# mika314/melonix

Hardware: AMD Instinct MI355X
Metric: STFT+pitch+resynth frames/sec (48 kHz, 4096 FFT, 256 hop); % HBM roofline (higher is better)
Workload: dtype f32

## Files before the change

melonix_amd/csrc/capi_ctx.cpp:

```cpp
#include "capi_internal.h"
#include "stft_tables.h"

using namespace mx;

namespace mx {
namespace {
thread_local char g_err[512] = "";
}
int fail(int code, const char *fmt, ...) noexcept {
  va_list ap;
  va_start(ap, fmt);
  vsnprintf(g_err, sizeof(g_err), fmt, ap);
  va_end(ap);
  return code;
}

int default_frames_per_block(int N, int mode, int hop, int64_t count) {
  if (const char *e = getenv("MELONIX_FRAMES_PER_BLOCK")) {
    const int v = atoi(e);
    if (v > 0) return v;
  }
  const int cap = stft_frames_per_block_cap(N, mode, hop);
  const int64_t want_blocks = 2048;
  const int64_t want = std::max<int64_t>(1, std::min<int64_t>(cap, count / want_blocks));
  int g = 1;
  while (2 * g <= want) g *= 2;
  return g;
}

template <class P>
int build_tables(NTables &t) {
  constexpr int N = P::N;
  const auto tw2 = make_tw2<P>();
  const auto tw3 = make_tw3<P>();
  const auto ub = make_ubase<P>();
  HIP_TRY(hipMalloc(&t.tw2, tw2.size() * sizeof(float2)));
  HIP_TRY(hipMalloc(&t.tw3, tw3.size() * sizeof(float2)));
  HIP_TRY(hipMalloc(&t.ubase, ub.size() * sizeof(float2)));
  HIP_TRY(hipMemcpy(t.tw2, tw2.data(), tw2.size() * sizeof(float2), hipMemcpyHostToDevice));
  HIP_TRY(hipMemcpy(t.tw3, tw3.data(), tw3.size() * sizeof(float2), hipMemcpyHostToDevice));
  HIP_TRY(hipMemcpy(t.ubase, ub.data(), ub.size() * sizeof(float2), hipMemcpyHostToDevice));
  t.wext_host = make_wext(fold_scale(N));
  HIP_TRY(hipMalloc(&t.wext, t.wext_host.size() * sizeof(float)));
  HIP_TRY(hipMemcpy(t.wext, t.wext_host.data(), t.wext_host.size() * sizeof(float), hipMemcpyHostToDevice));
  return MX_OK;
}

int get_tables(mx_ctx *ctx, int N, NTables &out) {
  std::lock_guard<std::mutex> lk(ctx->mu);
  auto it = ctx->tables.find(N);
  if (it != ctx->tables.end()) {
    out = it->second;
    return MX_OK;
  }
  NTables t;
  int rc;
  switch (N) {
    case 4096: rc = build_tables<Plan<4096, kPlan4096E>>(t); break;
    case 16384: rc = build_tables<Plan<16384, 32>>(t); break;
    case 32768: rc = build_tables<Plan<32768, 32>>(t); break;
    default: return fail(MX_ERR_INVALID, "unsupported FFT size %d (supported: 4096, 16384, 32768)", N);
  }
  if (rc) return rc;
  ctx->tables[N] = t;
  out = t;
  return MX_OK;
}

int get_wtab(mx_ctx *ctx, int N, int hop, const NTables &nt, const float **out) {
  std::lock_guard<std::mutex> lk(ctx->mu);
  const auto key = std::make_pair(N, hop);
  auto it = ctx->wtabs.find(key);
  if (it != ctx->wtabs.end()) {
    *out = it->second;
    return MX_OK;
  }
  const std::vector<float> w = make_wtab(N, hop, nt.wext_host);
  float *d = nullptr;
  HIP_TRY(hipMalloc(&d, w.size() * sizeof(float)));
  HIP_TRY(hipMemcpy(d, w.data(), w.size() * sizeof(float), hipMemcpyHostToDevice));
  ctx->wtabs[key] = d;
  *out = d;
  return MX_OK;
}

int check_common(mx_ctx *ctx, const mx_audio *a, int N, int64_t count, int &kmin, int &kmax) {
  if (!ctx || !a) return fail(MX_ERR_INVALID, "null context or audio handle");
  if (N != 4096 && N != 16384 && N != 32768)
    return fail(MX_ERR_INVALID, "unsupported FFT size %d (supported: 4096, 16384, 32768)", N);
  if (count < 0) return fail(MX_ERR_INVALID, "negative frame count");
  if (kmin < 0 && kmax < 0) mx_pitch_band(N, 48000, &kmin, &kmax);
  kmin = std::max(kmin, 0);
  kmax = std::min(kmax, N / 2 - 1);
  if (kmin > kmax) return fail(MX_ERR_INVALID, "empty pitch band [%d,%d]", kmin, kmax);
  return MX_OK;
}

int stft_launch(mx_ctx *ctx, const mx_audio *a, int N, int mode, int hop, int64_t first_frame,
                const int32_t *d_ranges, int64_t count, int kmin, int kmax, float *d_mags,
                mx_pitch *d_pitch, uint8_t *d_rgb, float cmap_k, int run_length) {
  HIP_TRY(hipSetDevice(ctx->device));
  NTables t;
  int rc = get_tables(ctx, N, t);
  if (rc) return rc;
  StftArgs s{};
  s.audio = a->d_padded;
  s.n = a->n;
  s.wext = t.wext;
  s.decay = hop_decay(hop);
  s.tw2 = t.tw2;
  s.tw3 = t.tw3;
  s.ubase = t.ubase;
  s.ranges = d_ranges;
  s.hop = hop;
  s.first_frame = first_frame;
  s.count = count;
  s.kmin = kmin;
  s.kmax = kmax;
  s.mags = d_mags;
  s.pitch = d_pitch;
  s.rgb = d_rgb;
  s.cmap_k = cmap_k;
  s.frames_per_block = (mode != kRanges && ctx->frames_per_block > 0) ? ctx->frames_per_block
                       : run_length > 0                              ? run_length
                                                                     : default_frames_per_block(N, mode, hop, count);
  if (mode != kRanges) {
    rc = get_wtab(ctx, N, hop, t, &s.wtab);
    if (rc) return rc;
  }
  HIP_TRY(launch_stft(N, mode, s, ctx->stream));
  return MX_OK;
}

int64_t chunk_frames(int N) { return std::max<int64_t>(1, (int64_t)(1ull << 30) / ((int64_t)(N / 2) * 4)); }

void stage_trim(mx_ctx *ctx) {
  for (auto &st : ctx->stage)
    if (st.cap > ((size_t)256 << 20)) st.drop();
}

}

extern "C" {

const char *mx_last_error(void) { return g_err; }
#ifndef MX_SRC_SHA
#define MX_SRC_SHA "unknown"
#endif
const char *mx_version(void) { return "melonix_amd 0.1.0 gfx950 src:" MX_SRC_SHA; }

int mx_ctx_create(int device, mx_ctx **out) {
  return mx_guard([&]() -> int {
    if (!out) return fail(MX_ERR_INVALID, "out is null");
    *out = nullptr;
    int ndev = 0;
    hipError_t e = hipGetDeviceCount(&ndev);
    if (e != hipSuccess || ndev <= 0)
      return fail(MX_ERR_DEVICE, "no HIP device visible (%s); melonix_amd has no CPU path",
                  e == hipSuccess ? "device count is 0" : hipGetErrorString(e));
    if (device < 0 || device >= ndev) return fail(MX_ERR_INVALID, "device %d out of range [0,%d)", device, ndev);
    hipDeviceProp_t prop;
    HIP_TRY(hipGetDeviceProperties(&prop, device));
    if (strncmp(prop.gcnArchName, "gfx950", 6) != 0)
      return fail(MX_ERR_DEVICE, "device %d is %s; this library carries gfx950 (MI355X) code objects only", device,
                  prop.gcnArchName);
    HIP_TRY(hipSetDevice(device));
    mx_ctx *c = new (std::nothrow) mx_ctx();
    if (!c) return fail(MX_ERR_NOMEM, "out of host memory");
    c->device = device;
    e = hipStreamCreateWithFlags(&c->own_stream, hipStreamNonBlocking);
    if (e != hipSuccess) {
      delete c;
      return fail(MX_ERR_DEVICE, "hipStreamCreate: %s", hipGetErrorString(e));
    }
    c->stream = c->own_stream;
    *out = c;
    return MX_OK;
  });
}

void mx_ctx_destroy(mx_ctx *ctx) {
  mx_guard_void([&] {
    if (!ctx) return;
    hipSetDevice(ctx->device);
    hipStreamSynchronize(ctx->stream);
    for (auto &kv : ctx->tables) {
      hipFree(kv.second.tw2);
      hipFree(kv.second.tw3);
      hipFree(kv.second.ubase);
      hipFree(kv.second.wext);
    }
    for (auto &kv : ctx->wtabs) hipFree(kv.second);
    for (auto &st : ctx->stage) st.drop();
    for (auto &st : ctx->chain) st.drop();
    for (auto &st : ctx->f0dec) st.drop();
    pv_release(ctx);
    hipStreamDestroy(ctx->own_stream);
    delete ctx;
  });
}

int mx_ctx_set_stream(mx_ctx *ctx, void *hip_stream) {
  return mx_guard([&]() -> int {
    if (!ctx) return fail(MX_ERR_INVALID, "null context");
    ctx->stream = (hipStream_t)hip_stream;
    return MX_OK;
  });
}

int mx_ctx_use_own_stream(mx_ctx *ctx) {
  return mx_guard([&]() -> int {
    if (!ctx) return fail(MX_ERR_INVALID, "null context");
    ctx->stream = ctx->own_stream;
    return MX_OK;
  });
}

int mx_ctx_synchronize(mx_ctx *ctx) {
  return mx_guard([&]() -> int {
    if (!ctx) return fail(MX_ERR_INVALID, "null context");
    HIP_TRY(hipStreamSynchronize(ctx->stream));
    return MX_OK;
  });
}

int mx_ctx_release_scratch(mx_ctx *ctx) {
  return mx_guard([&]() -> int {
    if (!ctx) return fail(MX_ERR_INVALID, "null context");
    HIP_TRY(hipSetDevice(ctx->device));
    {
      std::lock_guard<std::mutex> lk(ctx->stage_mu);
      for (auto &st : ctx->stage) st.drop();
    }
    {
      std::lock_guard<std::mutex> lk(ctx->pv_mu);
      pv_release(ctx);
      ctx->pv_budget_auto = 0;
      ctx->pv_rec_full = false;
    }
    {
      std::lock_guard<std::mutex> lk(ctx->zc_mu);
      ctx->zc_scratch = ZcBitmaps{};
      for (auto &st : ctx->chain) st.drop();
    }
    {
      std::lock_guard<std::mutex> lk(ctx->f0_mu);
      for (auto &st : ctx->f0dec) st.drop();
    }
    return MX_OK;
  });
}

int mx_pinned_alloc(mx_ctx *ctx, size_t bytes, void **out) {
  return mx_guard([&]() -> int {
    if (!ctx || !out) return fail(MX_ERR_INVALID, "null context / out");
    *out = nullptr;
    if (bytes == 0) return MX_OK;
    HIP_TRY(hipSetDevice(ctx->device));
    const hipError_t e = hipHostMalloc(out, bytes, hipHostMallocDefault);
    if (e != hipSuccess) {
      *out = nullptr;
      return fail(MX_ERR_NOMEM, "hipHostMalloc(%zu): %s", bytes, hipGetErrorString(e));
    }
    return MX_OK;
  });
}

void mx_pinned_free(mx_ctx *ctx, void *p) {
  mx_guard_void([&] {
    if (!p) return;
    if (ctx) hipSetDevice(ctx->device);
    hipHostFree(p);
  });
}

int mx_ctx_set_frames_per_block(mx_ctx *ctx, int g) {
  return mx_guard([&]() -> int {
    if (!ctx || g < 0) return fail(MX_ERR_INVALID, "bad argument");
    ctx->frames_per_block = g;
    return MX_OK;
  });
}

int mx_audio_upload(mx_ctx *ctx, const float *host_wav, int64_t n, mx_audio **out) {
  return mx_guard([&]() -> int {
    if (!ctx || !out || n < 0 || (n > 0 && !host_wav)) return fail(MX_ERR_INVALID, "bad argument");
    if (n > 0x7fffffffLL - 2 * MX_AUDIO_PAD)
      return fail(MX_ERR_INVALID, "audio longer than the reference's int sample indices allow");
    HIP_TRY(hipSetDevice(ctx->device));
    mx_audio *a = new (std::nothrow) mx_audio();
    if (!a) return fail(MX_ERR_NOMEM, "out of host memory");
    const size_t total = (size_t)n + 2 * (size_t)MX_AUDIO_PAD;
    hipError_t e = hipMalloc(&a->d_padded, total * sizeof(float));
    if (e == hipSuccess) e = hipMemsetAsync(a->d_padded, 0, total * sizeof(float), ctx->stream);
    if (e == hipSuccess && n > 0)
      e = hipMemcpyAsync(a->d_padded + MX_AUDIO_PAD, host_wav, (size_t)n * sizeof(float), hipMemcpyHostToDevice,
                         ctx->stream);
    if (e == hipSuccess) e = hipStreamSynchronize(ctx->stream);
    if (e != hipSuccess) {
      if (a->d_padded) hipFree(a->d_padded);
      delete a;
      return fail(MX_ERR_DEVICE, "audio upload: %s", hipGetErrorString(e));
    }
    a->n = n;
    a->owned = true;
    *out = a;
    return MX_OK;
  });
}

int mx_audio_wrap_device(mx_ctx *ctx, const float *d_padded, int64_t n, mx_audio **out) {
  return mx_guard([&]() -> int {
    if (!ctx || !out || !d_padded || n < 0) return fail(MX_ERR_INVALID, "bad argument");
    if (reinterpret_cast<uintptr_t>(d_padded) & 15)
      return fail(MX_ERR_INVALID, "device audio buffer must be 16-byte aligned");
    mx_audio *a = new (std::nothrow) mx_audio();
    if (!a) return fail(MX_ERR_NOMEM, "out of host memory");
    a->d_padded = const_cast<float *>(d_padded);
    a->n = n;
    a->owned = false;
    *out = a;
    return MX_OK;
  });
}

int64_t mx_audio_length(const mx_audio *a) {
  return mx_guard([&]() -> int64_t {
    return a ? a->n : -1;
  });
}

int mx_audio_free(mx_ctx *ctx, mx_audio *a) {
  return mx_guard([&]() -> int {
    if (!a) return MX_OK;
    if (a->owned) {
      if (ctx) {
        hipSetDevice(ctx->device);
        hipStreamSynchronize(ctx->stream);
      }
      hipFree(a->d_padded);
    }
    delete a;
    return MX_OK;
  });
}
void mx_free(void *p) {
  mx_guard_void([&] {
    free(p);
  });
}

}
```

melonix_amd/csrc/kernels.h:

```cpp
#pragma once
#include <hip/hip_runtime.h>
#include <stdint.h>

#include "../../include/melonix_amd.h"

namespace mx {

enum StftMode {
  kBulkAligned = 0,
  kBulkAny = 1,
  kRanges = 2,
};

struct StftArgs {
  const float *audio;
  int64_t n;
  const float *wtab;
  const float *wext;
  float decay;
  const float2 *tw2;
  const float2 *tw3;
  const float2 *ubase;
  const int32_t *ranges;
  int hop;
  int64_t first_frame;
  int64_t count;
  int kmin, kmax;
  float *mags;
  mx_pitch *pitch;
  uint8_t *rgb;
  float cmap_k;
  int frames_per_block;
};

hipError_t launch_stft(int N, int mode, const StftArgs &a, hipStream_t s);
constexpr int kPlan4096E = 16;
int stft_points_per_thread(int N);
int stft_frames_per_block_cap(int N, int mode, int hop);

struct ResynthArgs {
  const float *audio;
  const mx_step *steps;
  int64_t nsteps;
  int64_t nsamples;
  float *pcm_f32;
  int16_t *pcm_i16;
};
hipError_t launch_resynth(const ResynthArgs &a, hipStream_t s);

struct PvArgs {
  const float *audio;
  int64_t n;
  double ratio;
  const int64_t *apos;
  const uint32_t *hop;
  const double *hratio;
  int64_t frames;
  const float *hann_scaled;
  const float *hann;
  const float2 *wsplit;
  const float2 *tw2, *tw3, *ubase;
  float2 *xrows;
  uint32_t *pkmap;
  uint32_t *pkcount;
  float *fthr;
  uint2 *recs;
  uint32_t rec_wg_cap;
  int rec_fpb_shift;
  uint32_t *rec_overflow;
  uint32_t *chunk_sums;
  uint16_t *chunk_org;
  uint32_t *group_sums;
  uint16_t *group_org;
  int scan_chunk;
  float *halo;
  float *s;
  int64_t s_len;
  float *pcm_f32;
  int16_t *pcm_i16;
  int64_t pcm_base;
  int frames_per_block;
  int64_t first;
  int global_first;
  const uint32_t *carry_in;
  uint32_t *carry_out;
  uint32_t *tot_sums;
  uint16_t *tot_org;
  const float *prev_tail;
  const float *next_head;
  const float *prev_final;
  int skip_head, skip_tail;
  int64_t out_lo, out_hi;
  int64_t s_origin;
  const double *tf, *rf;
  const int64_t *i0;
  int64_t frame_base;
  int sample_rate;
};
hipError_t launch_pv(const PvArgs &a, hipStream_t s);
hipError_t launch_pv_analyze(const PvArgs &a, hipStream_t s);
hipError_t launch_pv_synthesize(const PvArgs &a, hipStream_t s);
hipError_t launch_pv_analysis(const PvArgs &a, hipStream_t s);
hipError_t launch_pv_maps(const PvArgs &a, hipStream_t s);
hipError_t launch_pv_offsets(const PvArgs &a, hipStream_t s);
hipError_t launch_pv_synthesis(const PvArgs &a, hipStream_t s);
hipError_t launch_pv_finish(const PvArgs &a, hipStream_t s);
int64_t pv_halo_floats(int64_t frames);
hipError_t launch_pv_compose_maps(const uint32_t *sums, const uint16_t *org, int64_t n, uint32_t *out_sums, uint16_t *out_org, hipStream_t s,
                                  int sums_stride = 0, int org_stride = 0);
hipError_t launch_pv_resample(const PvArgs &a, hipStream_t s);
hipError_t launch_pv_edge_sum(float *dst, const float *x, const float *y, int n, hipStream_t s);
hipError_t launch_pv_plan_const(int64_t *apos, uint32_t *hop, double *hratio, int64_t rows, int64_t fbase, double r,
                                hipStream_t s);

struct F0Args {
  const float *audio;
  int hop;
  int64_t first_frame;
  int64_t count;
  int tau_min, tau_max;
  float threshold;
  const float2 *tw2, *tw3, *ubase;
  mx_f0 *out;
  int frames_per_block;
  mx_f0_cand *cands;
  int sample_rate;
};
hipError_t launch_f0(const F0Args &a, hipStream_t s);

struct F0DecodeArgs {
  const mx_f0 *track;
  const mx_f0_cand *cands;
  int64_t count;
  int64_t q_unvoiced, q_jump, q_switch;
  int32_t max_jump_cents;
  int64_t chunk;
  uint16_t *bp;
  int64_t *prod;
  uint16_t *map;
  mx_f0 *out;
  uint8_t *state;
};
int64_t f0_decode_default_chunk(int64_t count);
hipError_t launch_f0_decode(const F0DecodeArgs &a, hipStream_t s);
hipError_t launch_colormap(const float *mags, uint8_t *rgb, int64_t nbins_total, float k, hipStream_t s);

hipError_t launch_picks(const float *audio_padded, int64_t n, float *d_out, int64_t *counts, int *nlevels, hipStream_t s);

hipError_t launch_zc_bitmaps(const float *audio_padded, int64_t n, uint64_t *zc7, uint64_t *zc3,
                             hipStream_t s);

size_t grain_rank_scratch_bytes(int64_t n);
hipError_t launch_grain_rank(const float *audio_padded, int64_t n, const uint64_t *zc7, const uint64_t *zc3, void *rank_scratch,
                             hipStream_t s);
void grain_chain_sizes(int64_t n, uint32_t nodes, int *levels_out, uint32_t *out_cap_out, size_t *bytes_out);
hipError_t launch_grain_chain(const float *audio_padded, int64_t n, const uint64_t *zc7, const uint64_t *zc3, void *rank_scratch,
                              uint32_t nodes, void *chain_scratch, int32_t **d_starts, int32_t **d_lens, float **d_firsts,
                              hipStream_t s);

}
```

melonix_amd/csrc/stft_kernel_impl.h:

```cpp
#pragma once
#include <hip/hip_runtime.h>

#include "colormap_core.h"
#include "kernels.h"
#include "stft_core.h"
#include "stft_tables.h"

#define MX_BARRIER() __syncthreads()

namespace mx {

template <bool MAXOP>
__device__ __forceinline__ unsigned wave_reduce_u32(unsigned k) {
  constexpr unsigned ident = MAXOP ? 0u : 0xffffffffu;
#define MX_DPP_STEP(CTRL, ROWS)                                                                      \
  {                                                                                                  \
    const unsigned o = (unsigned)__builtin_amdgcn_update_dpp((int)ident, (int)k, CTRL, ROWS, 0xf, false); \
    k = MAXOP ? (o > k ? o : k) : (o < k ? o : k);                                                   \
  }
  MX_DPP_STEP(0xB1, 0xf)
  MX_DPP_STEP(0x4E, 0xf)
  MX_DPP_STEP(0x141, 0xf)
  MX_DPP_STEP(0x140, 0xf)
  MX_DPP_STEP(0x142, 0xa)
  MX_DPP_STEP(0x143, 0xc)
#undef MX_DPP_STEP
  return (unsigned)__builtin_amdgcn_readlane((int)k, 63);
}
__device__ __forceinline__ unsigned long long wave_max_u64(unsigned long long k) {
  const unsigned hi = (unsigned)(k >> 32), lo = (unsigned)k;
  const unsigned mhi = wave_reduce_u32<true>(hi);
  const unsigned long long tie = __ballot(hi == mhi);
  unsigned mlo;
  if (__builtin_popcountll(tie) == 1) mlo = (unsigned)__builtin_amdgcn_readlane((int)lo, __builtin_ctzll(tie));
  else mlo = wave_reduce_u32<true>(hi == mhi ? lo : 0u);
  return ((unsigned long long)mhi << 32) | mlo;
}

template <int IMM, bool NT = true>
__device__ __forceinline__ void st_row_nt(const float *base, unsigned off, float x) {
  static_assert(IMM >= -4096 && IMM <= 4095, "global_store immediate offset");
#if defined(__HIP_DEVICE_COMPILE__)
  if constexpr (NT) asm volatile("global_store_dword %0, %1, %2 offset:%3 nt" : : "v"(off), "v"(x), "s"(base), "n"(IMM) : "memory");
  else asm volatile("global_store_dword %0, %1, %2 offset:%3" : : "v"(off), "v"(x), "s"(base), "n"(IMM) : "memory");
#endif
}

template <class P, int MODE, int HOP, int WPE, bool DEFER = false, bool PREFETCH = false, bool CMAP = false, bool DIRECT = false,
          bool CIRC = false>
__global__ __launch_bounds__(P::T) __attribute__((amdgpu_waves_per_eu(WPE, WPE)))
void stft_kernel(const StftArgs a0) {
  const StftArgs &a = a0;
  using C = P;
  constexpr int N = P::N;
  constexpr int NW = C::T / 64;
  constexpr int kRed = (NW > 1) ? ((NW + 1) / 2) * 2 : 0;
  constexpr bool kTw3Bases = (P::R3 == 16);
  constexpr int kTw2 = ((C::TW2 + 1) / 2) * 2;
  static_assert(P::R3 == 16 || P::R3 == 8, "twiddle placement per plan");
  static_assert(!DIRECT || (NW > 1 && !DEFER && !CMAP), "direct row stores: multi-wave, non-deferred plans");
  static_assert(!CIRC || (MODE != kRanges && HOP == 0 && !PREFETCH && !CMAP), "circular window: bulk modes");
  constexpr int IMG = t1_size<C>();
  __shared__ __attribute__((aligned(16))) float2 lds[IMG + kRed + (DEFER ? C::M / 2 : 0) + kTw2];
  float *const lout = reinterpret_cast<float *>(DEFER ? lds + IMG + kRed : lds);
  float2 *const ltw2 = lds + IMG + kRed + (DEFER ? C::M / 2 : 0);

  const int t_ = threadIdx.x;
  const bool wave0 = __builtin_amdgcn_readfirstlane(t_) < 64;
  cpx u[kTw3Bases ? 1 : P::R3];
  cpx ulo;
  cpx w3r[kTw3Bases ? 1 : P::R3 - 1], w3base[6];
  if constexpr (kTw3Bases) {
    cpx uhi_unused;
    post_bases<P>(t_, a.ubase, ulo, uhi_unused);
    fetch_tw3_bases<P>(t_, a.tw3, w3base);
  } else {
    post_twiddles<P>(t_, a.ubase, *reinterpret_cast<cpx(*)[P::R3]>(&u));
    fetch_tw3<P>(t_, a.tw3, *reinterpret_cast<cpx(*)[P::R3 - 1]>(&w3r));
  }
  const uint32_t bmask_ = band_mask<P>(t_, a.kmin, a.kmax);
  uint32_t umask = 0;
#pragma unroll
  for (int o = 0; o < P::E; ++o) umask |= (__ballot((bmask_ >> o) & 1u) != 0ull) ? (1u << o) : 0u;
  umask = __builtin_amdgcn_readfirstlane(umask);
  constexpr bool kSlide = (MODE == kBulkAligned) && (HOP > 0) && Slide<P, (HOP > 0 ? HOP : 2)>::ok;
  constexpr int SD = Slide<P, (HOP > 0 ? HOP : 2)>::D;
  constexpr float kSc = 0.5f / (float)N;
  for (int i = t_; i < C::TW2; i += C::T) ltw2[i] = a.tw2[i];
  MX_BARRIER();

  unsigned lb = blockIdx.x;
  {
    const unsigned nb = gridDim.x, xcd = lb & 7u, q = nb >> 3, r = nb & 7u;
    lb = (xcd < r ? xcd * (q + 1) : r * (q + 1) + (xcd - r) * q) + (lb >> 3);
  }
  const int64_t f0 = (int64_t)lb * a.frames_per_block;
  const int64_t f1 = (f0 + a.frames_per_block < a.count) ? f0 + a.frames_per_block : a.count;

  cpx Y[P::E];
  cpx edge[SD], nx[SD];
  if constexpr (kSlide) {
    const int64_t e0 = (a.first_frame + f0 + 1) * (int64_t)HOP;
    if (f0 < f1) load_frame<P, 1, true>(t_, Y, a.audio + MX_AUDIO_PAD + (e0 - N), a.wtab);
    slide_edge<P, HOP>(t_, a.wtab, 2.0f * (float)N, edge);
  }

  unsigned long long *const red = reinterpret_cast<unsigned long long *>(lds + IMG);
  auto flush_pitch = [&](int64_t fr, int tt) {
    if (a.pitch && tt == 0) {
      unsigned long long b = red[0];
#pragma unroll
      for (int i = 1; i < NW; ++i) b = red[i] > b ? red[i] : b;
      mx_pitch p;
      p.bin = 0x7fffffff - (int)(unsigned)(b & 0xffffffffull);
      p.mag = __uint_as_float((unsigned)(b >> 32));
      a.pitch[fr] = p;
    }
  };
  const bool want_rows = a.mags != nullptr || (CMAP && a.rgb != nullptr);
  auto flush_row = [&](int64_t fr, int tt) {
    if (want_rows) {
      using f32x4 = float __attribute__((ext_vector_type(4)));
      const f32x4 *l4 = reinterpret_cast<const f32x4 *>(lout) + tt;
      f32x4 *row4 = reinterpret_cast<f32x4 *>(a.mags + (size_t)fr * (size_t)(N / 2)) + tt;
      f32x4 q[C::M / 4 / C::T];
#pragma unroll
      for (int i = 0; i < C::M / 4 / C::T; ++i) q[i] = l4[C::T * i];
      if (!CMAP || a.mags) {
#pragma unroll
        for (int i = 0; i < C::M / 4 / C::T; ++i) {
          __builtin_nontemporal_store(q[i], &row4[C::T * i]);
        }
      }
      if constexpr (CMAP) {
        if (a.rgb) {
          uint32_t *trow = reinterpret_cast<uint32_t *>(a.rgb + (size_t)fr * (size_t)(N / 2) * 3) + 3 * tt;
#pragma unroll 1
          for (int i = 0; i < C::M / 4 / C::T; ++i) {
            uint32_t w3[3];
            texel4(q[i].x, q[i].y, q[i].z, q[i].w, a.cmap_k, w3);
            uint32_t *o = trow + 3 * C::T * i;
            o[0] = w3[0];
            o[1] = w3[1];
            o[2] = w3[2];
          }
        }
      }
    }
  };

  auto frame_ptrs = [&](int64_t fr, int zo, const float *&x, const float *&w) {
    if constexpr (MODE == kRanges) {
      const int s = a.ranges[2 * fr], e = a.ranges[2 * fr + 1];
      const bool outside = (e <= 0) || ((int64_t)e - N >= a.n);
      x = outside ? a.audio : a.audio + MX_AUDIO_PAD + ((int64_t)e - N);
      int64_t d0 = (int64_t)N - ((int64_t)e - (int64_t)s);
      d0 = d0 < (int64_t)(N - 1 - kWOff) ? (int64_t)(N - 1 - kWOff) : d0;
      d0 = d0 > (int64_t)(kWDmax + kWTail) ? (int64_t)(kWDmax + kWTail) : d0;
      w = a.wext + kWOff + d0;
    } else {
      const int64_t e = (a.first_frame + fr + 1) * (int64_t)a.hop;
      x = a.audio + MX_AUDIO_PAD + (e - N);
      w = a.wtab + zo;
    }
  };
  float cpx_[2 * Circ<P>::CS], cpw_[2 * Circ<P>::CS];
  if constexpr (CIRC) {
    if (f0 < f1) {
      const int64_t pe = (a.first_frame + f0 + 1) * (int64_t)a.hop;
      circ_load_first<P>(t_, Y, a.audio + MX_AUDIO_PAD + (pe - N), a.wtab, circ_geo<P>(pe, a.hop).o);
    }
  }
  cpx xr[(PREFETCH && !kSlide) ? P::E : 1];
  if constexpr (PREFETCH && !kSlide) {
    if (f0 < f1) {
      const float *x0;
      const float *w0;
      frame_ptrs(f0, 0, x0, w0);
      load_raw<P, (MODE == kBulkAligned)>(t_, xr, x0);
    }
  }

  for (int64_t f = f0; f < f1; ++f) {
    int t = t_;
    unsigned bmask = bmask_;
    int zoff = 0;
    asm volatile("" : "+v"(t), "+v"(bmask), "+s"(zoff));
    int out_lo, out_hi;
    out_bases<P>(t, out_lo, out_hi);

    if constexpr (CIRC) {
      if (f > f0) {
        const int64_t pe = (a.first_frame + f + 1) * (int64_t)a.hop;
        const CircGeo<P> geo = circ_geo<P>(pe, a.hop);
        circ_fetch<P>(t, a.audio + MX_AUDIO_PAD + (pe - 2 * (int64_t)a.hop), a.wtab + zoff + (N - 2 * a.hop), geo, cpx_, cpw_);
        circ_step<P>(t, Y, a.decay, geo, cpx_, cpw_);
      }
    } else if constexpr (kSlide) {
      if (f > f0) slide_step<P, HOP>(Y, nx, edge, a.decay, kSc);
      if (f + 1 < f1) slide_fetch<P, HOP>(t, a.audio + MX_AUDIO_PAD + (a.first_frame + f + 2) * (int64_t)HOP, nx);
    } else {
      const float *x;
      const float *w;
      frame_ptrs(f, zoff, x, w);
      if constexpr (PREFETCH) {
        if constexpr (MODE == kRanges) apply_window<P, -1, false>(t, Y, xr, w);
        else apply_window_geo<P>(t, Y, xr, a.wtab + N + zoff, a.hop);
      } else if constexpr (MODE == kRanges) {
        load_frame<P, -1, false>(t, Y, x, w);
      } else {
        load_frame_geo<P, (MODE == kBulkAligned)>(t, Y, x, a.wtab + N + zoff, a.hop);
      }
    }

    cpx v[P::E];
    pass1<P>(Y, v);
    constexpr bool kTw2Batch = (P::NB2 == 1);
    store_t1<P>(t, v, lds);
    MX_BARRIER();
    if constexpr (DEFER || DIRECT) {
      if (f > f0) flush_pitch(f - 1, t);
    }
    if constexpr (kTw2Batch) {
      cpx w2[P::R2 - 1];
      load_t1_tw2<P>(t, v, lds, ltw2, w2);
      if constexpr (DEFER) {
        if (f > f0) flush_row(f - 1, t);
      }
      MX_BARRIER();
      pass2_reg<P>(v, w2);
    } else {
      load_t1<P>(t, v, lds);
      if constexpr (DEFER) {
        if (f > f0) flush_row(f - 1, t);
      }
      MX_BARRIER();
      pass2<P>(t, v, ltw2);
    }
    store_t2<P>(t, v, lds);
    MX_BARRIER();
    load_t2<P>(t, v, lds);
    MX_BARRIER();
    float mg[P::E];
    if (NW == 1 || wave0) {
      if constexpr (kTw3Bases) {
        pass3_bases<P, true>(t, v, w3base);
        post_fly<P, true>(t, v, ulo, csel(t == 0, mk(-1.0f, 0.0f), ulo), mg);
      } else {
        pass3_reg<P, true>(t, v, *reinterpret_cast<cpx(*)[P::R3 - 1]>(&w3r));
        post<P, true>(t, v, *reinterpret_cast<cpx(*)[P::R3]>(&u), mg);
      }
    } else {
      if constexpr (kTw3Bases) {
        pass3_bases<P, false>(t, v, w3base);
        post_fly<P, false>(t, v, ulo, ulo, mg);
      } else {
        pass3_reg<P, false>(t, v, *reinterpret_cast<cpx(*)[P::R3 - 1]>(&w3r));
        post<P, false>(t, v, *reinterpret_cast<cpx(*)[P::R3]>(&u), mg);
      }
    }

    if constexpr (PREFETCH && !kSlide) {
      if (f + 1 < f1) {
        const float *xn;
        const float *wn;
        frame_ptrs(f + 1, zoff, xn, wn);
        load_raw<P, (MODE == kBulkAligned)>(t, xr, xn);
      }
    }

    unsigned long long best = 0ull;
    if (a.pitch) {
      const unsigned klo = 0x7fffffffu - (unsigned)out_lo, khi = 0x7fffffffu - (unsigned)out_hi;
      const unsigned nlo = 0x7fffffffu - (unsigned)(C::M - out_lo), nhi = 0x7fffffffu - (unsigned)(C::M - out_hi);
#pragma unroll
      for (int s = 0; s < C::R3; ++s) {
        constexpr int H = C::R3 / 2;
        if (!((umask >> (2 * s)) & 3u)) continue;
        const unsigned b0 = (s < H ? klo : khi) - (unsigned)(C::NS3 * s);
        unsigned b1 = (s < H ? nlo : nhi) + (unsigned)(C::NS3 * s);
        if (s == H) b1 = (t == 0) ? 0x7fffffffu - (unsigned)(C::M / 2) : b1;
        const unsigned v0 = (unsigned)((int)(bmask << (31 - 2 * s)) >> 31);
        const unsigned v1 = (unsigned)((int)(bmask << (31 - (2 * s + 1))) >> 31);
        const unsigned long long k0 = ((unsigned long long)(__float_as_uint(mg[2 * s]) & v0) << 32) | (b0 & v0);
        const unsigned long long k1 = ((unsigned long long)(__float_as_uint(mg[2 * s + 1]) & v1) << 32) | (b1 & v1);
        best = k0 > best ? k0 : best;
        best = k1 > best ? k1 : best;
      }
      best = wave_max_u64(best);
      if constexpr (NW > 1) {
        if ((t & 63) == 0) red[t >> 6] = best;
      }
    }

    if constexpr (DIRECT) {
      if (want_rows) {
        const float *row = a.mags + (size_t)f * (size_t)(N / 2);
        constexpr int H = C::R3 / 2;
        constexpr int STEP = 4 * C::NS3;
        constexpr int G = 8192 / STEP;
        static_assert((STEP == 4096 || STEP == 2048) && H % G == 0, "slot groups share an offset through the store's immediate");
        const unsigned blo = 4u * (unsigned)out_lo, bhi = 4u * (unsigned)(out_hi + C::NS3 * H);
        const unsigned nlo = 4u * (unsigned)(C::M - out_lo), nhi = 4u * (unsigned)(C::M - out_hi - C::NS3 * H);
        static_for<0, C::R3>([&](auto ss) {
          constexpr int s = decltype(ss)::value;
          constexpr int sl = s < H ? s : s - H;
          constexpr int su = (sl & ~(G - 1)) + G / 2, sd = (sl & ~(G - 1)) + G / 2 - 1;
          const unsigned o0 = (s < H ? blo : bhi) + (unsigned)(su * STEP);
          unsigned o1 = (s < H ? nlo : nhi) - (unsigned)(sd * STEP);
          if constexpr (s == H) {
            o1 = (t == 0) ? (unsigned)(4 * (C::M / 2)) + (unsigned)((sl - sd) * STEP) : o1;
          }
          st_row_nt<(sl - su) * STEP>(row, o0, mg[2 * s]);
          st_row_nt<-(sl - sd) * STEP, false>(row, o1, mg[2 * s + 1]);
        });
      }
    } else if (want_rows) {
      float *plo = lout + out_lo, *phi = lout + out_hi;
      float *mlo = lout + (C::M - out_lo), *mhi = lout + (C::M - out_hi);
#pragma unroll
      for (int s = 0; s < C::R3; ++s) {
        constexpr int H = C::R3 / 2;
        (s < H ? plo : phi)[C::NS3 * s] = mg[2 * s];
        if (s == H) (t == 0 ? lout + C::M / 2 : mhi - C::NS3 * H)[0] = mg[2 * s + 1];
        else (s < H ? mlo : mhi)[-C::NS3 * s] = mg[2 * s + 1];
      }
    }
    if constexpr (!DEFER && !DIRECT) {
      if (want_rows) {
        MX_BARRIER();
        flush_row(f, t);
        MX_BARRIER();
      } else {
        MX_BARRIER();
      }
      if constexpr (NW > 1) {
        flush_pitch(f, t);
      } else if (a.pitch && t == 0) {
        mx_pitch p;
        p.bin = 0x7fffffff - (int)(unsigned)(best & 0xffffffffull);
        p.mag = __uint_as_float((unsigned)(best >> 32));
        a.pitch[f] = p;
      }
    }
  }
  if constexpr (DEFER || DIRECT) {
    if (f0 < f1) {
      MX_BARRIER();
      flush_pitch(f1 - 1, t_);
      if constexpr (DEFER) flush_row(f1 - 1, t_);
    }
  }
}


}
```

melonix_amd/csrc/stft_kernels.hip:

```cpp
#include <hip/hip_runtime.h>

#include "kernels.h"
#include "stft_kernel_impl.h"

namespace mx {

namespace {

template <class P>
struct Tune {
  static constexpr bool TWO_WAVE = (P::E == 16);
  static constexpr int WPE = TWO_WAVE ? 3 : 2;
  static constexpr bool PREFETCH = (P::E == 32);
  static constexpr bool slides(int hop) {
    return P::N == 4096 ? (hop == 256 || hop == 512) : P::N == 16384 ? (hop == 512 || hop == 1024) : hop == 1024;
  }
  static constexpr bool DIRECT = (P::N >= 16384);
  static constexpr bool CIRC = (P::N >= 16384);
  static constexpr bool DEFER = TWO_WAVE;
};

template <class P, int HOP>
bool try_slide(const StftArgs &b, dim3 grid, dim3 block, hipStream_t s) {
  if constexpr (Slide<P, HOP>::ok && Tune<P>::slides(HOP)) {
    if (b.hop != HOP) return false;
    hipLaunchKernelGGL((stft_kernel<P, kBulkAligned, HOP, Tune<P>::WPE, Tune<P>::DEFER, false, false, Tune<P>::DIRECT>),
                       grid, block, 0, s, b);
    return true;
  } else {
    return false;
  }
}

template <class P>
bool try_circ(const StftArgs &b, dim3 grid, dim3 block, hipStream_t s) {
  if constexpr (!Tune<P>::CIRC) {
    return false;
  } else {
    if (!Circ<P>::ok(b.hop)) return false;
    hipLaunchKernelGGL((stft_kernel<P, kBulkAny, 0, Tune<P>::WPE, Tune<P>::DEFER, false, false, Tune<P>::DIRECT, true>),
                       grid, block, 0, s, b);
    return true;
  }
}

template <class P>
hipError_t launch_plan(int mode, const StftArgs &a, hipStream_t s) {
  if (a.count <= 0) return hipSuccess;
  const int g = a.frames_per_block > 0 ? a.frames_per_block : 1;
  const int64_t blocks = (a.count + g - 1) / g;
  if (blocks > 0x7fffffffLL) return hipErrorInvalidValue;
  StftArgs b = a;
  b.frames_per_block = g;
  const dim3 grid((unsigned)blocks), block(P::T);
  constexpr int W = Tune<P>::WPE;
  constexpr bool DF = Tune<P>::DEFER, PF = Tune<P>::PREFETCH, DR = Tune<P>::DIRECT;
  switch (mode) {
    case kBulkAligned:
      if (!(try_slide<P, 256>(b, grid, block, s) || try_slide<P, 512>(b, grid, block, s) ||
            try_slide<P, 1024>(b, grid, block, s) || try_circ<P>(b, grid, block, s)))
        hipLaunchKernelGGL((stft_kernel<P, kBulkAligned, 0, W, DF, PF, false, DR>), grid, block, 0, s, b);
      break;
    case kBulkAny:
      if (try_circ<P>(b, grid, block, s)) break;
      hipLaunchKernelGGL((stft_kernel<P, kBulkAny, 0, W, DF, PF, false, DR>), grid, block, 0, s, b); break;
    case kRanges:
      if (a.rgb) hipLaunchKernelGGL((stft_kernel<P, kRanges, 0, (W > 2 ? 2 : W), DF, false, true>), grid, block, 0, s, b);
      else hipLaunchKernelGGL((stft_kernel<P, kRanges, 0, W, DF, false, false, DR>), grid, block, 0, s, b);
      break;
    default: return hipErrorInvalidValue;
  }
  return hipGetLastError();
}

}

int stft_points_per_thread(int N) { return N == 4096 ? kPlan4096E : 32; }

int stft_frames_per_block_cap(int N, int mode, int hop) {
  if (N == 32768 && mode != kRanges && Tune<Plan<32768, 32>>::CIRC && !Tune<Plan<32768, 32>>::slides(hop) &&
      Circ<Plan<32768, 32>>::ok(hop))
    return 32;
  return N == 32768 ? 8 : (N == 4096 ? 32 : 16);
}

hipError_t launch_stft(int N, int mode, const StftArgs &a, hipStream_t s) {
  switch (N) {
    case 4096: return launch_plan<Plan<4096, kPlan4096E>>(mode, a, s);
    case 16384: return launch_plan<Plan<16384, 32>>(mode, a, s);
    case 32768: return launch_plan<Plan<32768, 32>>(mode, a, s);
  }
  return hipErrorInvalidValue;
}

}
```

Baseline: 337.1 million.

## Launch sliding STFT as persistent spans sized to resident occupancy

For the 4096-point sliding-window kernels, the grid is capped at the number of blocks that can be resident at once, queried through the occupancy API. Each block then processes a contiguous span of frames in 8-frame units instead of one fixed frames_per_block group. At each frames_per_block boundary the block reloads a full window so the sliding recurrence resets at the same points as before. A block whose span starts mid-group replays the missing slide steps to reach its start. This removes tail-wave imbalance and block launch overhead, at the cost of extra replay work and more kernel complexity.

Result: slower. 319.8 million (-5.1%).

```diff
diff --git a/melonix_amd/csrc/capi_ctx.cpp b/melonix_amd/csrc/capi_ctx.cpp
--- a/melonix_amd/csrc/capi_ctx.cpp
+++ b/melonix_amd/csrc/capi_ctx.cpp
@@ -26,6 +26,14 @@
   int g = 1;
   while (2 * g <= want) g *= 2;
   return g;
+}
+
+int default_span_slots() {
+  if (const char *e = getenv("MELONIX_STFT_SLOTS")) {
+    const int v = atoi(e);
+    if (v >= 0) return v;
+  }
+  return -1;
 }
 
 template <class P>
@@ -124,6 +132,7 @@
   s.frames_per_block = (mode != kRanges && ctx->frames_per_block > 0) ? ctx->frames_per_block
                        : run_length > 0                              ? run_length
                                                                      : default_frames_per_block(N, mode, hop, count);
+  s.span_slots = default_span_slots();
   if (mode != kRanges) {
     rc = get_wtab(ctx, N, hop, t, &s.wtab);
     if (rc) return rc;
diff --git a/melonix_amd/csrc/kernels.h b/melonix_amd/csrc/kernels.h
--- a/melonix_amd/csrc/kernels.h
+++ b/melonix_amd/csrc/kernels.h
@@ -31,7 +31,11 @@
   uint8_t *rgb;
   float cmap_k;
   int frames_per_block;
+  int span_slots;
+  int64_t span_q;
+  int span_r;
 };
+constexpr int kSpanUnit = 8;
 
 hipError_t launch_stft(int N, int mode, const StftArgs &a, hipStream_t s);
 constexpr int kPlan4096E = 16;
diff --git a/melonix_amd/csrc/stft_kernel_impl.h b/melonix_amd/csrc/stft_kernel_impl.h
--- a/melonix_amd/csrc/stft_kernel_impl.h
+++ b/melonix_amd/csrc/stft_kernel_impl.h
@@ -47,7 +47,7 @@
 }
 
 template <class P, int MODE, int HOP, int WPE, bool DEFER = false, bool PREFETCH = false, bool CMAP = false, bool DIRECT = false,
-          bool CIRC = false>
+          bool CIRC = false, bool SPANS = false>
 __global__ __launch_bounds__(P::T) __attribute__((amdgpu_waves_per_eu(WPE, WPE)))
 void stft_kernel(const StftArgs a0) {
   const StftArgs &a = a0;
@@ -60,6 +60,7 @@
   static_assert(P::R3 == 16 || P::R3 == 8, "twiddle placement per plan");
   static_assert(!DIRECT || (NW > 1 && !DEFER && !CMAP), "direct row stores: multi-wave, non-deferred plans");
   static_assert(!CIRC || (MODE != kRanges && HOP == 0 && !PREFETCH && !CMAP), "circular window: bulk modes");
+  static_assert(!SPANS || ((MODE == kBulkAligned) && Slide<P, (HOP > 0 ? HOP : 2)>::ok), "spans: the sliding kernels");
   constexpr int IMG = t1_size<C>();
   __shared__ __attribute__((aligned(16))) float2 lds[IMG + kRed + (DEFER ? C::M / 2 : 0) + kTw2];
   float *const lout = reinterpret_cast<float *>(DEFER ? lds + IMG + kRed : lds);
@@ -94,15 +95,43 @@
     const unsigned nb = gridDim.x, xcd = lb & 7u, q = nb >> 3, r = nb & 7u;
     lb = (xcd < r ? xcd * (q + 1) : r * (q + 1) + (xcd - r) * q) + (lb >> 3);
   }
-  const int64_t f0 = (int64_t)lb * a.frames_per_block;
-  const int64_t f1 = (f0 + a.frames_per_block < a.count) ? f0 + a.frames_per_block : a.count;
+  int64_t f0 = (int64_t)lb * a.frames_per_block;
+  int64_t f1 = f0 + a.frames_per_block;
+  if constexpr (SPANS) {
+    if (a.span_q > 0) {
+      const unsigned big0 = gridDim.x - (unsigned)a.span_r;
+      const int64_t u0 = (int64_t)lb * a.span_q + (lb > big0 ? (int64_t)(lb - big0) : 0);
+      f0 = u0 * kSpanUnit;
+      f1 = (u0 + a.span_q + (lb >= big0 ? 1 : 0)) * kSpanUnit;
+    }
+  }
+  f1 = f1 < a.count ? f1 : a.count;
 
   cpx Y[P::E];
   cpx edge[SD], nx[SD];
+  int run_left = 0;
   if constexpr (kSlide) {
-    const int64_t e0 = (a.first_frame + f0 + 1) * (int64_t)HOP;
-    if (f0 < f1) load_frame<P, 1, true>(t_, Y, a.audio + MX_AUDIO_PAD + (e0 - N), a.wtab);
     slide_edge<P, HOP>(t_, a.wtab, 2.0f * (float)N, edge);
+    if (f0 < f1) {
+      const int into = (SPANS && a.span_q > 0) ? (int)(f0 % a.frames_per_block) : 0;
+      const float *xe = a.audio + MX_AUDIO_PAD + (a.first_frame + (f0 - into) + 1) * (int64_t)HOP;
+      load_frame<P, 1, true>(t_, Y, xe - N, a.wtab);
+      if constexpr (SPANS) {
+        constexpr int kReplay = 8;
+        cpx rx[kReplay][SD];
+#pragma unroll 1
+        for (int j = 0; j < into; j += kReplay) {
+#pragma unroll
+          for (int k = 0; k < kReplay; ++k)
+            if (j + k < into) slide_fetch<P, HOP>(t_, xe + (k + 1) * HOP, rx[k]);
+#pragma unroll
+          for (int k = 0; k < kReplay; ++k)
+            if (j + k < into) slide_step<P, HOP>(Y, rx[k], edge, a.decay, kSc);
+          xe += kReplay * HOP;
+        }
+      }
+      run_left = a.frames_per_block - into;
+    }
   }
 
   unsigned long long *const red = reinterpret_cast<unsigned long long *>(lds + IMG);
@@ -197,8 +226,17 @@
         circ_step<P>(t, Y, a.decay, geo, cpx_, cpw_);
       }
     } else if constexpr (kSlide) {
-      if (f > f0) slide_step<P, HOP>(Y, nx, edge, a.decay, kSc);
-      if (f + 1 < f1) slide_fetch<P, HOP>(t, a.audio + MX_AUDIO_PAD + (a.first_frame + f + 2) * (int64_t)HOP, nx);
+      if (f > f0) {
+        if (SPANS && run_left == 0) {
+          load_frame<P, 1, true>(t, Y, a.audio + MX_AUDIO_PAD + ((a.first_frame + f + 1) * (int64_t)HOP - N), a.wtab + zoff);
+          run_left = a.frames_per_block;
+        } else {
+          slide_step<P, HOP>(Y, nx, edge, a.decay, kSc);
+        }
+      }
+      if (f + 1 < f1 && (!SPANS || run_left != 1))
+        slide_fetch<P, HOP>(t, a.audio + MX_AUDIO_PAD + (a.first_frame + f + 2) * (int64_t)HOP, nx);
+      --run_left;
     } else {
       const float *x;
       const float *w;
diff --git a/melonix_amd/csrc/stft_kernels.hip b/melonix_amd/csrc/stft_kernels.hip
--- a/melonix_amd/csrc/stft_kernels.hip
+++ b/melonix_amd/csrc/stft_kernels.hip
@@ -1,4 +1,7 @@
 #include <hip/hip_runtime.h>
+
+#include <algorithm>
+#include <atomic>
 
 #include "kernels.h"
 #include "stft_kernel_impl.h"
@@ -18,14 +21,44 @@
   static constexpr bool DIRECT = (P::N >= 16384);
   static constexpr bool CIRC = (P::N >= 16384);
   static constexpr bool DEFER = TWO_WAVE;
+  static constexpr bool SPANS = TWO_WAVE;
 };
 
+template <class K>
+int resident_slots(K kernel, int threads) {
+  constexpr int kDevs = 64;
+  static std::atomic<int> cache[kDevs];
+  int dev = 0;
+  if (hipGetDevice(&dev) != hipSuccess || dev < 0 || dev >= kDevs) return 0;
+  int v = cache[dev].load(std::memory_order_relaxed);
+  if (v == 0) {
+    int per_cu = 0, cus = 0;
+    if (hipOccupancyMaxActiveBlocksPerMultiprocessor(&per_cu, kernel, threads, 0) != hipSuccess ||
+        hipDeviceGetAttribute(&cus, hipDeviceAttributeMultiprocessorCount, dev) != hipSuccess) {
+      (void)hipGetLastError();
+      per_cu = 0;
+    }
+    v = (per_cu > 0 && cus > 0) ? std::max(8, per_cu * cus / 8 * 8) : -1;
+    cache[dev].store(v, std::memory_order_relaxed);
+  }
+  return v > 0 ? v : 0;
+}
+
 template <class P, int HOP>
-bool try_slide(const StftArgs &b, dim3 grid, dim3 block, hipStream_t s) {
+bool try_slide(const StftArgs &b0, dim3 grid, dim3 block, hipStream_t s) {
   if constexpr (Slide<P, HOP>::ok && Tune<P>::slides(HOP)) {
-    if (b.hop != HOP) return false;
-    hipLaunchKernelGGL((stft_kernel<P, kBulkAligned, HOP, Tune<P>::WPE, Tune<P>::DEFER, false, false, Tune<P>::DIRECT>),
-                       grid, block, 0, s, b);
+    if (b0.hop != HOP) return false;
+    const auto kernel =
+        stft_kernel<P, kBulkAligned, HOP, Tune<P>::WPE, Tune<P>::DEFER, false, false, Tune<P>::DIRECT, false, Tune<P>::SPANS>;
+    StftArgs b = b0;
+    const int64_t slots = !Tune<P>::SPANS ? 0 : b.span_slots < 0 ? resident_slots(kernel, P::T) : b.span_slots;
+    if (slots > 0 && (int64_t)grid.x > slots) {
+      const int64_t units = (b.count + kSpanUnit - 1) / kSpanUnit, g = std::min(slots, units);
+      b.span_q = units / g;
+      b.span_r = (int)(units % g);
+      grid.x = (unsigned)g;
+    }
+    hipLaunchKernelGGL(kernel, grid, block, 0, s, b);
     return true;
   } else {
     return false;
@@ -52,6 +85,8 @@
   if (blocks > 0x7fffffffLL) return hipErrorInvalidValue;
   StftArgs b = a;
   b.frames_per_block = g;
+  b.span_q = 0;
+  b.span_r = 0;
   const dim3 grid((unsigned)blocks), block(P::T);
   constexpr int W = Tune<P>::WPE;
   constexpr bool DF = Tune<P>::DEFER, PF = Tune<P>::PREFETCH, DR = Tune<P>::DIRECT;
```
